# raznem/spp-rl

Measured on AMD Instinct MI355X. Metric: env-steps/sec (rollout+update) SPP-SAC Hopper-v2, higher is better.
Workload: dtype fp32

## Files before the change

include/spprl.h:

```cpp
#ifndef SPPRL_H
#define SPPRL_H
#include <stdint.h>

#ifdef __cplusplus
extern "C" {
#endif

typedef int sppStatus;
enum {
  SPP_OK = 0,
  SPP_E_INVALID_ARG = 1,
  SPP_E_SHAPE = 2,
  SPP_E_OOM = 3,
  SPP_E_HIP = 4,
  SPP_E_STATE = 5,
  SPP_E_RCCL = 6
};

const char* sppGetLastError(void);
int sppGetVersion(void);

typedef struct sppMT19937* sppMTHandle;
sppStatus sppMTCreate(sppMTHandle* out, uint32_t seed);
sppStatus sppMTRandint(sppMTHandle h, int64_t high, int64_t n, int64_t* out_host);
// ... 122 lines not shown
enum { SPP_BUCKET_CRITIC = 0, SPP_BUCKET_ACTOR = 1, SPP_BUCKET_ACM = 2, SPP_BUCKET_ALL = 3 };
sppStatus sppAllReduceGrads(sppAgentHandle h, int bucket, int world, void* rccl_comm, void* stream);
sppStatus sppCommAllReduceSum(void* rccl_comm, void* buf_dev, int64_t count, int dtype, void* stream);
sppStatus sppCommAllGather(void* rccl_comm, const void* send_dev, void* recv_dev, int64_t bytes, void* stream);

sppStatus sppAcmRegressStep(sppAgentHandle h, const float* x, const float* y, int B, float* loss_dev,
                            void* stream);
sppStatus sppAcmRegressGrads(sppAgentHandle h, const float* x, const float* y, int B, float* loss_dev,
                             void* stream);
sppStatus sppAcmRegressApply(sppAgentHandle h, void* stream);
sppStatus sppAcmSgd(sppAgentHandle h, const float* x_dev, const float* y_dev, int nsteps, int bs, float* loss_sum,
                    void* stream);
sppStatus sppAcmSgdEpoch(sppAgentHandle h, const float* x_dev, const float* y_dev, int nrows, int bs,
                         float* loss_sum, void* stream);
sppStatus sppAcmSgdStatus(sppAgentHandle h, int* timed_out_host);
sppStatus sppAcmSgdStatusAsync(sppAgentHandle h, int* timed_out_pinned, void* stream);
int sppAcmSgdMaxBatch(sppAgentHandle h);
int sppAcmSgdWorkgroups(sppAgentHandle h, int bs);
sppStatus sppReplayGatherAcm(sppReplayHandle h, const int64_t* idx_dev, int B, float* x, float* y, void* stream);
sppStatus sppReplaySetAcmColumns(sppReplayHandle h, const int* cols_host, int n);

sppStatus sppAgentSetTiming(sppAgentHandle h, int enable);
sppStatus sppAgentStageSplit(sppAgentHandle h, int* bits_out);
sppStatus sppAgentGetTiming(sppAgentHandle h, double* ms_out , int64_t* count_out );

sppStatus sppPolicyAct(sppAgentHandle h, const float* obs , int E, const float* eps ,
                       const float* noise , float act_noise, int mode, int denormalize_actor_out,
                       float* target_state_out , float* env_action_out , void* stream);

sppStatus sppSynthEnvStep(const float* A , const float* obs , const float* action ,
                          int E, int ob, int ac, float* next_obs, float* reward, void* stream);

sppStatus sppRandUniform(float* out_dev, int64_t n, const float* lo_dev, const float* hi_dev, int period,
                         uint64_t seed, uint64_t offset, void* stream);
sppStatus sppEpisodeAccum(const float* rew, const uint8_t* end, int E, float* ep_ret, double* sums, void* stream);
sppStatus sppSynthEnvReset(float* obs , const uint8_t* mask, int E, int ob, uint64_t seed,
                           uint64_t offset, void* stream);

sppStatus sppObsNormalize(const float* x, int64_t rows, int ob, const float* lo, const float* hi, const float* mean,
                          const float* std, int min_max, int inverse, float* out, void* stream);

sppStatus sppGaeScan(const float* rew, const float* v, const float* v_next, const uint8_t* done,
                     const uint8_t* end, int64_t T, int64_t E, double gamma, double lam, int mode, float* q_out,
                     float* adv, void* stream);
sppStatus sppPpoClipLoss(const float* lp_old, const float* lp_new, const float* adv, int B, float eps, float* grad,
                         float* out2, void* stream);
// ... 61 lines not shown
```

spp-rl_amd/csrc/api.hip:

```cpp
#include <dlfcn.h>
#include <stdarg.h>
#include <stdio.h>
#include <string.h>

#include <algorithm>
#include <memory>
#include <string>
#include <vector>

#include "../../include/spprl.h"
#include "internal.h"
#include "layout.h"
#include "replay.h"
#include "sac_kernels.h"
#include "host.h"

#include "optim.hip"
#include "replay.hip"
#include "stats.hip"
#include "sac.hip"
#include "ddpg.hip"
#include "kset.h"
#ifdef SPP_SINGLE_TU
#include "ks_dw.hip"
// ... 683 lines not shown
  DevArray<PackJob> d_pj;
  std::vector<TabSeg> tab;
  int tab_floats = 0;
  ActorDev actor{};
  CriticDev critic[2]{}, targ[2]{};
  AcmDev acm{};
  const float4* acm_W1n = nullptr;
  BAcmDev bacm{};
  ActorDev actor_targ{};
  const float4 *bacm_W1n = nullptr, *bacm_W21n = nullptr;
  BAcmScratch bz{};
  float *RBH = nullptr, *RBH1 = nullptr, *RS21 = nullptr, *RBP1 = nullptr, *RPZ = nullptr, *RPZ21 = nullptr;
  DevArray<float> scratch;
  float *S = nullptr, *S2 = nullptr, *ACT = nullptr, *AENV = nullptr, *R = nullptr, *DN = nullptr, *EPS1 = nullptr,
        *EPS2 = nullptr;
  float *H1[2] = {}, *H2[2] = {}, *D1[2] = {}, *D2[2] = {}, *DQ[2] = {};
  float *AH1 = nullptr, *AH2 = nullptr, *AD1 = nullptr, *AD2 = nullptr, *ADH = nullptr;
  float *Z1 = nullptr, *Z2 = nullptr, *T3 = nullptr, *part = nullptr;
  float *aux = nullptr;
  float* GAD = nullptr;
  uint64_t* MASK = nullptr;
  bool minq_split = false;
  int stage_split = 0;
  float *THD = nullptr, *SCA = nullptr, *SLP = nullptr;
  AcmScratch mq{};
  float *RX = nullptr, *RZ1 = nullptr, *RZ2 = nullptr, *RP1 = nullptr, *RP2 = nullptr, *RP3 = nullptr;
  DwSet dws[2];
  DevArray<AdamJob> d_adam;
  int cur_B = -1;
  float* w3p[2] = {};
  int64_t w3p_stride = 0;
  float* alpha_grad = nullptr;
  DevArray<float> sgd_slab;
  DevArray<int> sgd_sync;
  int sgd_max_wg = -1;
  bool timing = false;
  std::vector<hipEvent_t> tev[5];
  size_t tused[5] = {0, 0, 0, 0, 0};
};

static void tmark(sppAgent* a, int kind, hipStream_t st) {
  if (!a->timing) return;
  auto& v = a->tev[kind];
  if (a->tused[kind] == v.size()) {
    hipEvent_t e;
    hipEventCreate(&e);
// ... 360 lines not shown
  for (int i = 0; i < (a->ddpg ? 1 : 2); ++i) {
    NetBufs& n = a->net[SPP_NET_CRITIC1 + i];
    jobs[i] = AdamJob{n.p, n.g, n.m, n.v, a->net[SPP_NET_CRITIC1_TARG + i].p, n.n};
  }
  NetBufs& na = a->net[SPP_NET_ACTOR];
  jobs[2] = AdamJob{na.p, na.g, na.m, na.v, a->ddpg ? a->net[SPP_NET_ACTOR_TARG].p : nullptr, na.n};
  NetBufs& nm = a->net[SPP_NET_ACM];
  jobs[3] = AdamJob{nm.p, nm.g, nm.m, nm.v, nullptr, nm.n};
  if (!a->d_adam.ptr) SPP_CHECK_HIP(a->d_adam.alloc(4));
  SPP_CHECK_HIP(hipMemcpy(a->d_adam.ptr, jobs, sizeof(jobs), hipMemcpyHostToDevice));
  return SPP_OK;
}

static void launch_adam(sppAgent* a, int first, int count, int64_t n, int64_t step, float lr, float tau,
                        hipStream_t st) {
  const double bc1 = 1.0 - std::pow(0.9, (double)step), bc2s = std::sqrt(1.0 - std::pow(0.999, (double)step));
  hipLaunchKernelGGL(k_adam, dim3(std::max(1, std::min(cdiv(n, 256 * 4), 1024)), count), dim3(256), 0, st,
                     (const AdamJob*)(a->d_adam.ptr + first), (float)(-(lr / bc1)), (float)bc2s, tau);
}

constexpr int kStageWGPerCU = 3;
constexpr int kStageSplitAll = 7;
constexpr int kStageSplitDefault = kStageSplitAll;
static int stage_grid(sppAgent* a, int Bp) {
  return std::max(1, std::min(cdiv(Bp / 32, kWavesPerWG), kStageWGPerCU * a->num_cu));
}

static SacArgs make_args(sppAgent* a, int B) {
  SacArgs p{};
  p.B = B;
  p.Bp = (int)round_up(B, 32);
  p.inv_B = 1.f / (float)B;
  p.S = a->S; p.S2 = a->S2; p.ACT = a->ACT; p.AENV = a->AENV; p.R = a->R; p.DN = a->DN;
  p.EPS1 = a->EPS1; p.EPS2 = a->EPS2;
  p.min_max = a->cfg.min_max_denormalize;
  p.lo = a->lo; p.hi = a->hi; p.mean = a->mean; p.std = a->std;
  p.actor_lim = a->limits.ptr;
  p.acm_lim = a->limits.ptr + a->cfg.aout;
  p.gamma = a->cfg.gamma;
  p.custom_loss = a->cfg.custom_loss;
  p.norm_closs = a->cfg.norm_closs;
  p.alpha = a->alpha_f32;
  p.actor = a->actor;
  for (int i = 0; i < 2; ++i) {
    p.critic[i] = a->critic[i];
    p.targ[i] = a->targ[i];
// ... 75 lines not shown
  KernelSet ks;
  SPP_REQUIRE(find_kset(cfg->algo, cfg->ob, cfg->aout, cfg->ac, cfg->acm_critic != 0, cfg->mlp_bf16 != 0, &ks),
              SPP_E_SHAPE, "no kernel instantiation for algo %d (ob=%d, aout=%d, ac=%d, bf16=%d)", cfg->algo, cfg->ob,
              cfg->aout, cfg->ac, cfg->mlp_bf16);
  SPP_CHECK_HIP(hipSetDevice(device));
  auto a = std::make_unique<sppAgent>();
  a->cfg = *cfg;
  a->device = device;
  a->ks = ks;
  hipDeviceProp_t prop;
  SPP_CHECK_HIP(hipGetDeviceProperties(&prop, device));
  a->num_cu = prop.multiProcessorCount;
  {
    const char* t = getenv("SPP_SAC_TEAM");
    a->team_ok = !(t && t[0] == '0');
    const char* m = getenv("SPP_MINQ_SPLIT");
    a->minq_split = ks.actor_fwd && ks.actor_minq && ks.actor_bwd && !(m && m[0] == '0');
    const char* g = getenv("SPP_STAGE_SPLIT");
    const int want = g ? atoi(g) : kStageSplitDefault;
    const bool tab_fits = 128 + 3 * round_up(std::max(cfg->aout, 1), 32) + round_up(std::max(cfg->ac, 1), 32) <= kStageTab;
    const bool have = ks.heads_stage && ks.trunk_bwd && ks.trunk_fwd_a && ks.squash_a && ks.critics_a &&
                      ks.trunk_fwd_c && ks.squash_c && ks.critic_rest;
    if (a->minq_split && have && tab_fits) a->stage_split = want & kStageSplitAll;
  }
  const int ob = cfg->ob, aout = cfg->aout, ac = cfg->ac;
  a->cin = ob + (cfg->acm_critic ? ac : aout);
  a->ddpg = cfg->algo == SPP_ALGO_DDPG_ACM || cfg->algo == SPP_ALGO_DDPG;
  a->plain = cfg->algo == SPP_ALGO_SAC || cfg->algo == SPP_ALGO_DDPG;
  const bool dd = a->ddpg;
  a->lay[SPP_NET_ACTOR] = dd ? ddpg_actor_layout(ob, aout) : sac_actor_layout(ob, aout);
  if (dd) a->lay[SPP_NET_ACTOR_TARG] = a->lay[SPP_NET_ACTOR];
  a->lay[SPP_NET_CRITIC1] = a->lay[SPP_NET_CRITIC1_TARG] = critic_layout(a->cin);
  if (!dd) a->lay[SPP_NET_CRITIC2] = a->lay[SPP_NET_CRITIC2_TARG] = critic_layout(a->cin);
  if (!dd) a->lay[SPP_NET_ACM] = acm_layout(2 * ob, ac);
  else if (!a->plain) a->lay[SPP_NET_ACM] = bacm_layout(2 * ob, ac);
  a->Bmax = cfg->max_batch;
  const int64_t Bp = round_up(cfg->max_batch, 32);
  SPP_REQUIRE((int64_t)Bp * 256 * 4 < ((int64_t)1 << 31), SPP_E_SHAPE, "max_batch %d too large (31-bit buffer offsets)",
              cfg->max_batch);
  a->Bpmax = (int)Bp;
  const int64_t ntiles = Bp / 32;
  const int64_t per = Bp;
  int64_t total = 0;
  auto take = [&](int64_t rows) { int64_t o = total; total += rows * per; return o; };
  const int64_t oS = take(ob), oS2 = take(ob), oACT = take(aout), oAENV = take(ac), oR = take(1), oDN = take(1),
                oE1 = take(aout), oE2 = take(aout);
// ... 150 lines not shown
  hipLaunchKernelGGL(k_stage_batch, dim3(cdiv(s.Bp, 256)), dim3(256), 0, st, s);
  a->cur_B = bt->B;
  return SPP_OK;
}

static sppStatus critic_grads_staged(sppAgentHandle a, float* losses, hipStream_t st) {
  SPP_REQUIRE(!a->ddpg, SPP_E_STATE, "not a SAC_AcM agent");
  const int B = a->cur_B;
  SPP_REQUIRE(B > 0, SPP_E_STATE, "no staged batch");
  sppStatus s = check_ready(a);
  if (s) return s;
  if (a->dws[0].B != B) {
    s = build_dw(a, 0, B);
    if (s) return s;
  }
  launch_pack(a, PJ_ACTOR, PJ_LISTS, st);
  SacArgs p = make_args(a, B);
  const int grid = sac_critic_grid(a, p.Bp);
  tmark(a, 0, st);
  const bool team = phase_team(a, p.Bp);
  if (!team && (a->stage_split & 4)) {
    hipLaunchKernelGGL(a->ks.trunk_fwd_c, dim3(tile_grid(a, p.Bp)), dim3(256), 0, st, p, a->mq);
    hipLaunchKernelGGL(a->ks.squash_c, dim3(stage_grid(a, p.Bp)), dim3(256), 0, st, stage_args(a, p), a->mq);
    hipLaunchKernelGGL(a->ks.critic_rest, dim3(grid), dim3(256), 0, st, p);
  } else {
    hipLaunchKernelGGL(team ? a->ks.critic_team : a->ks.critic, dim3(grid), dim3(team ? 64 * kTeamCritic : 256), 0, st, p);
  }
  tmark(a, 0, st);
  SPP_CHECK_HIP(hipGetLastError());
  tmark(a, 2, st);
  launch_dw(a, 0, 0, st);
  tmark(a, 2, st);
  hipLaunchKernelGGL(k_finalize_critic, dim3(1), dim3(kFinThreads), 0, st, (const float*)a->part, p.Bp / 32, B, losses);
  SPP_CHECK_HIP(hipGetLastError());
  return SPP_OK;
}

sppStatus sppSacAcmCriticGrads(sppAgentHandle a, const sppBatch* bt, const float* eps_next, float* losses,
                               void* stream) {
  SPP_REQUIRE(a, SPP_E_INVALID_ARG, "null");
  if (bt) {
    sppStatus s = stage(a, bt, eps_next, nullptr, S(stream));
    if (s) return s;
  } else if (eps_next) {
    const int Bp = (int)round_up(a->cur_B, 32);
    SPP_REQUIRE(a->cur_B > 0, SPP_E_STATE, "no staged batch");
    hipLaunchKernelGGL(k_eps_copy_fm, dim3(cdiv((int64_t)a->cfg.aout * Bp, 256)), dim3(256), 0, S(stream), eps_next,
// ... 7 lines not shown
  a->steps[1] += 1;
  tmark(a, 3, S(stream));
  launch_adam(a, 0, 2, a->net[SPP_NET_CRITIC1].n, a->steps[1], a->cfg.critic_lr, a->cfg.tau, S(stream));
  tmark(a, 3, S(stream));
  SPP_CHECK_HIP(hipGetLastError());
  return SPP_OK;
}

static sppStatus actor_grads(sppAgentHandle a, float* losses, hipStream_t st) {
  SPP_REQUIRE(!a->ddpg, SPP_E_STATE, "not a SAC_AcM agent");
  const int B = a->cur_B;
  SPP_REQUIRE(B > 0, SPP_E_STATE, "no staged batch");
  launch_pack(a, PJ_CRITIC, PJ_LISTS, st);
  SacArgs p = make_args(a, B);
  AcmScratch z{a->Z1, a->Z2, a->T3, a->GAD, a->MASK};
  const int grid = tile_grid(a, p.Bp);
  tmark(a, 1, st);
  const bool team = phase_team(a, p.Bp);
  if (!team && a->minq_split) {
    z = a->mq;
    if (a->stage_split & 2) {
      hipLaunchKernelGGL(a->ks.trunk_fwd_a, dim3(grid), dim3(256), 0, st, p, z);
      hipLaunchKernelGGL(a->ks.squash_a, dim3(stage_grid(a, p.Bp)), dim3(256), 0, st, stage_args(a, p), z);
      hipLaunchKernelGGL(a->ks.critics_a, dim3(grid), dim3(256), 0, st, p, z);
    } else {
      hipLaunchKernelGGL(a->ks.actor_fwd, dim3(grid), dim3(256), 0, st, p, z);
    }
    hipLaunchKernelGGL(k_minq_scan, dim3(1), dim3(kMinqScanThreads), 0, st, (const uint32_t*)z.CNT, z.OFF, z.NG, p.Bp / 32);
    hipLaunchKernelGGL(k_minq_scatter, dim3(cdiv(p.Bp, 256)), dim3(256), 0, st, (const uint8_t*)z.SEL,
                       (const uint32_t*)z.OFF, z.LIST[0], z.LIST[1], p.Bp);
    hipLaunchKernelGGL(a->ks.actor_minq, dim3(grid), dim3(256), 0, st, p, z);
    if (a->stage_split & 1) {
      hipLaunchKernelGGL(a->ks.heads_stage, dim3(stage_grid(a, p.Bp)), dim3(256), 0, st, stage_args(a, p), z);
      hipLaunchKernelGGL(a->ks.trunk_bwd, dim3(grid), dim3(256), 0, st, p, z);
    } else {
      hipLaunchKernelGGL(a->ks.actor_bwd, dim3(grid), dim3(256), 0, st, p, z);
    }
  } else {
    hipLaunchKernelGGL(team ? a->ks.actor_team : a->ks.actor, dim3(grid), dim3(team ? 64 * kTeamActor : 256), 0, st, p, z);
    if (a->ks.actor_heads) hipLaunchKernelGGL(a->ks.actor_heads, dim3(grid), dim3(256), 0, st, p, z);
  }
  tmark(a, 1, st);
  SPP_CHECK_HIP(hipGetLastError());
  tmark(a, 2, st);
  launch_dw(a, 0, 1, st);
  tmark(a, 2, st);
  hipLaunchKernelGGL(k_actor_partials, dim3(1), dim3(kFinThreads), 0, st, (const float*)a->part, p.Bp / 32, B, a->cfg.aout,
                     a->cfg.custom_loss, (double)a->cfg.target_entropy, a->alpha_grad ? a->alpha_grad : a->aux,
                     losses);
  SPP_CHECK_HIP(hipGetLastError());
  return SPP_OK;
}

sppStatus sppSacAcmActorGrads(sppAgentHandle a, const float* eps_cur, float* losses, void* stream) {
  SPP_REQUIRE(a, SPP_E_INVALID_ARG, "null");
  const int B = a->cur_B;
  SPP_REQUIRE(B > 0, SPP_E_STATE, "no staged batch");
  const int Bp = (int)round_up(B, 32);
  if (eps_cur)
    hipLaunchKernelGGL(k_eps_copy_fm, dim3(cdiv((int64_t)a->cfg.aout * Bp, 256)), dim3(256), 0, S(stream), eps_cur,
                       a->EPS2, a->cfg.aout, B, Bp);
  return actor_grads(a, losses, S(stream));
}

sppStatus sppAgentStageSplit(sppAgentHandle a, int* bits_out) {
  SPP_REQUIRE(a && bits_out, SPP_E_INVALID_ARG, "null");
  *bits_out = a->stage_split;
  return SPP_OK;
}

sppStatus sppAgentBindAlphaGrad(sppAgentHandle a, float* g) {
  SPP_REQUIRE(a, SPP_E_INVALID_ARG, "null");
  a->alpha_grad = g;
  return SPP_OK;
}

sppStatus sppSacAcmDrawEps(sppAgentHandle a, uint64_t seed, uint64_t counter, void* stream) {
  SPP_REQUIRE(a && a->cur_B > 0, SPP_E_STATE, "no staged batch");
  const int B = a->cur_B, Bp = (int)round_up(B, 32);
  SPP_REQUIRE((int64_t)a->cfg.aout * Bp < ((int64_t)1 << 31), SPP_E_SHAPE, "draw_eps: aout * Bp >= 2^31");
  const int64_t quads = (int64_t)a->cfg.aout * Bp / 4;
  hipLaunchKernelGGL(k_eps_fm, dim3(cdiv(quads, 256), 2), dim3(256), 0, S(stream), a->EPS1, a->cfg.aout, B, Bp, seed,
                     2 * counter, a->EPS2, 2 * counter + 1);
  SPP_CHECK_HIP(hipGetLastError());
  return SPP_OK;
}

sppStatus sppAgentReadEps(sppAgentHandle a, int which, float* out, void* stream) {
  SPP_REQUIRE(a && out && (which == 0 || which == 1), SPP_E_INVALID_ARG, "read_eps: bad args");
  SPP_REQUIRE(a->cur_B > 0, SPP_E_STATE, "no staged batch");
// ... 621 lines not shown
```

spp-rl_amd/csrc/kset.h:

```cpp
#pragma once
#include "sac.hip"
#include "sac_bf.h"
#include "ddpg.hip"
#include "sac_team.h"
#include "ddpg_team.h"

namespace spp {

struct KernelSet {
  void (*critic)(SacArgs);
  void (*actor)(SacArgs, AcmScratch);
  void (*actor_heads)(SacArgs, AcmScratch);
  void (*act)(SacArgs, ActArgs);
  void (*acmreg)(SacArgs, AcmRegArgs);
  void (*dcritic)(SacArgs, BAcmScratch);
  void (*dactor)(SacArgs, BAcmScratch);
  void (*dact)(SacArgs, ActArgs, BAcmScratch);
  void (*dreg)(SacArgs, BAcmRegArgs);
  void (*critic_team)(SacArgs);
  void (*actor_team)(SacArgs, AcmScratch);
  void (*act_team)(SacArgs, ActArgs);
  void (*dcritic_team)(SacArgs, BAcmScratch);
  void (*dactor_team)(SacArgs, BAcmScratch);
  void (*dact_team)(SacArgs, ActArgs, BAcmScratch);
  void (*actor_fwd)(SacArgs, AcmScratch);
  void (*actor_minq)(SacArgs, AcmScratch);
  void (*actor_bwd)(SacArgs, AcmScratch);
  void (*heads_stage)(SacArgs, AcmScratch);
  void (*trunk_bwd)(SacArgs, AcmScratch);
  void (*trunk_fwd_a)(SacArgs, AcmScratch);
  void (*squash_a)(SacArgs, AcmScratch);
  void (*critics_a)(SacArgs, AcmScratch);
  void (*trunk_fwd_c)(SacArgs, AcmScratch);
  void (*squash_c)(SacArgs, AcmScratch);
  void (*critic_rest)(SacArgs);
};

template <int OB, int AOUT, int AC, bool ACMC, bool BF = false>
KernelSet make_kset() {
  using C = Cfg<OB, AOUT, AC, ACMC, BF>;
  void (*heads)(SacArgs, AcmScratch) = nullptr;
  if constexpr (C::NB_PAIR > 2) heads = k_sac_actor_heads<C>;
  void (*critic)(SacArgs) = k_sac_critic_phase<C>;
#if SPP_BF16_TWO_TILES
  if constexpr (C::BF && C::ACMC && !C::F3) critic = k_sac_critic_phase2<C>;
#endif
  KernelSet ks{critic, k_sac_actor_phase<C>, heads, k_policy_act<C>, k_acm_regress<C>,
               nullptr, nullptr, nullptr, nullptr};
  if constexpr (!C::BF) {
    ks.actor_fwd = k_sac_actor_phase<C, true>;
    ks.actor_minq = k_sac_minq_backward<C>;
    ks.actor_bwd = k_sac_actor_heads<C, true>;
    if constexpr (C::NB_PAIR <= 2) {
      ks.heads_stage = k_sac_heads_stage<C>;
      ks.trunk_bwd = k_sac_actor_trunk_bwd<C>;
      ks.trunk_fwd_a = k_sac_trunk_fwd<C, true>;
      ks.squash_a = k_sac_squash_stage<C, true>;
      ks.critics_a = k_sac_actor_phase<C, true, true>;
      ks.trunk_fwd_c = k_sac_trunk_fwd<C, false>;
      ks.squash_c = k_sac_squash_stage<C, false>;
      ks.critic_rest = k_sac_critic_phase<C, true>;
    }
  }
  return ks;
}
template <int OB, int AOUT, int AC, bool ACMC>
KernelSet make_dkset() {
  using D = DCfg<OB, AOUT, AC, ACMC>;
  return {nullptr, nullptr, nullptr, nullptr, nullptr,
          k_ddpg_critic_phase<D>, k_ddpg_actor_phase<D>, k_ddpg_policy_act<D>, k_bacm_regress<D>};
}

#define SPP_KSET_CASE(mk, o, a, c)                                     \
  if (ob == o && aout == a && ac == c) {                               \
    *ks = acmc ? mk<o, a, c, true>() : mk<o, a, c, false>();           \
    return true;                                                       \
  }

bool kset_sac_hopper(int ob, int aout, int ac, bool acmc, KernelSet* ks);
bool kset_sac_hcheetah(int ob, int aout, int ac, bool acmc, KernelSet* ks);
bool kset_sac_ant(int ob, int aout, int ac, bool acmc, KernelSet* ks);
bool kset_sac_small(int ob, int aout, int ac, bool acmc, KernelSet* ks);
bool kset_ddpg(int ob, int aout, int ac, bool acmc, KernelSet* ks);
bool kset_ddpg_ant(int ob, int aout, int ac, bool acmc, KernelSet* ks);
// ... 6 lines not shown
```

spp-rl_amd/csrc/sac.hip:

```cpp
#pragma once
#include "sac_kernels.h"

namespace spp {

constexpr float kLog2 = 0.69314718055994530942f;
constexpr float kLogSqrt2Pi = 0.91893853320467274178f;

template <int OB_, int AOUT_, int AC_, bool ACMC_, bool BF_ = false>
struct Cfg {
  static constexpr int OB = OB_, AOUT = AOUT_, AC = AC_;
  static constexpr bool ACMC = ACMC_;
  static constexpr bool BF = BF_;
  static constexpr bool F3 = !BF_ || SPP_BF16_FUSE3;
  static constexpr int NB_OB = blocks_of(OB);
  static constexpr int NB_AOUT = blocks_of(AOUT);
  static constexpr int NB_H2 = blocks_of(2 * AOUT);
  static constexpr int NB_PAIR = (AOUT + 15) / 16;
  static constexpr int CA = ACMC ? AC : AOUT;
  static constexpr int NB_CA = blocks_of(CA);
  static constexpr int NB_CIN = NB_OB + NB_CA;
  static constexpr int NB_ACMIN = NB_OB + NB_AOUT;
  static constexpr uint64_t RV_X = rv_nat(OB, NB_OB);
  static constexpr uint64_t RV_H = rv_nat(256, 8);
  static constexpr uint64_t RV_CIN = rv_cat(OB, NB_OB, CA, NB_CA);
// ... 457 lines not shown
        const float u = fadd_rn(mu, fmul_rn(e, sc));
        float lpj;
        if constexpr (F) {
          lpj = -0.5f * e * e - ls - kLogSqrt2Pi;
        } else {
          const float d = fsub_rn(u, mu);
          const float var = fmul_rn(sc, sc);
          lpj = fsub_rn(fsub_rn(fdiv_rn(-fmul_rn(d, d), 2.f * var), logf(sc)), kLogSqrt2Pi);
        }
        const float cj = 2.f * fsub_rn(fsub_rn(kLog2, u), t_softplus<F>(-2.f * u));
        lp += ok ? lpj : 0.f;
        corr += ok ? cj : 0.f;
        const float a = fmul_rn(t_tanh<F>(u), actor_lim<true>(p, L.tbl, jj));
        const float ad = denorm<true>(p, L.tbl, jj, a);
        if (ok) L.pl[j0 * 32] = ad;
      }
    }
  SPP_XLANE_SYNC();
  const float tot = lp + __shfl_xor(lp, 32, 64);
  const float tc = corr + __shfl_xor(corr, 32, 64);
  return fsub_rn(tot, tc);
}

template <class C, bool STAGED = false>
__global__ __launch_bounds__(256, 1) void k_sac_critic_phase(SacArgs p) {
  __shared__ __attribute__((aligned(16))) float smem[kWavesPerWG * kLdsPerWave];
  __shared__ __attribute__((aligned(16))) float tbl[kTabMax];
  __shared__ __attribute__((aligned(16))) float s_dq[kWavesPerWG][32];
  SPP_TP_INIT();
  load_table(p, tbl);
  const int w = threadIdx.x >> 6, lane = threadIdx.x & 63;
  float* big = smem + w * kLdsPerWave;
  float* small = big + kSmallRow * 32;
  const int ntiles = p.Bp / 32;
  const int ld = p.Bp;
  const float alpha = *p.alpha;
  float w3a[4] = {0.f, 0.f, 0.f, 0.f}, w3b[4] = {0.f, 0.f, 0.f, 0.f}, b3a = 0.f, b3b = 0.f;
  for (int tile = blockIdx.x * kWavesPerWG + w; tile < ntiles; tile += gridDim.x * kWavesPerWG) {
    const Lane L = make_lane(big, small, tbl, ld, tile * 32 + (lane & 31));
    const int b = L.b;
    const bool valid = b < p.B;
    uint64_t d0 = 0, d1 = 0, d2 = 0, d3 = 0;
    float lp2;
    f32x16 tin[C::NB_CIN];
    if constexpr (STAGED) {
      SPP_TP(0);
      load_cat_gg<C::NB_OB, C::NB_CA>(tin, p.S2, C::OB, p.SCA, C::CA, L.ld4, L.vo);
      lp2 = p.SLP[b];
    } else {
      SPP_TP(0);
      actor_trunk<C, false>(p.actor, p.S2, C::OB * L.ld4, L, nullptr, nullptr, d0, d1, d2, d3);
      {
        f32x16 hd[C::NB_PAIR];
        load_pair<C>(hd, big);
        lp2 = squash_write<C, true>(p, hd, p.EPS1, L);
      }
      SPP_TP(4);
      if constexpr (C::ACMC) {
        f32x16 xin[C::NB_ACMIN];
        load_cat_gl<C::NB_OB, C::NB_AOUT>(xin, p.S2, C::OB * L.ld4, C::OB, L.ld4, L.vo, big, C::AOUT);
        acm_forward<C, false>(p, xin, L, nullptr, nullptr, nullptr);
        load_cat_gl<C::NB_OB, C::NB_CA>(tin, p.S2, C::OB * L.ld4, C::OB, L.ld4, L.vo, small, C::AC);
      } else {
        load_cat_gl<C::NB_OB, C::NB_CA>(tin, p.S2, C::OB * L.ld4, C::OB, L.ld4, L.vo, big, C::AOUT);
      }
    }
    SPP_TP(5);
    const float q1t = critic_forward<C, false, 6>(p.targ[0], tin, L, nullptr, nullptr, d0, d1, d2, d3);
    const float q2t = critic_forward<C, false, 8>(p.targ[1], tin, L, nullptr, nullptr, d0, d1, d2, d3);
    const float notdone = 1.f - p.DN[b];
    const float y = fadd_rn(p.R[b], fmul_rn(p.gamma * notdone, fsub_rn(fminf(q1t, q2t), alpha * lp2)));
    float lq0 = 0.f, lq1 = 0.f;
#pragma unroll 1
    for (int i = 0; i < 2; ++i) {
      uint64_t m1lo = 0, m1hi = 0, m2lo = 0, m2hi = 0;
      f32x16 xin[C::NB_CIN];
      load_cat_gg<C::NB_OB, C::NB_CA>(xin, p.S, C::OB, C::ACMC ? p.AENV : p.ACT, C::CA, L.ld4, L.vo);
      const CriticDev& Q = p.critic[i];
      SPP_TP(10);
      const float q = critic_forward<C, true, 11, C::F3>(Q, xin, L, p.H1[i], C::F3 ? nullptr : p.H2[i], m1lo, m1hi,
                                                        m2lo, m2hi);
      const float diff = fsub_rn(q, y);
      const float dq = valid ? fmul_rn(2.f * diff, p.inv_B) : 0.f;
      const float lqi = (valid && L.h == 0) ? diff * diff : 0.f;
      if (i == 0) lq0 = lqi; else lq1 = lqi;
      if constexpr (!C::F3) {
        if (L.h == 0) p.DQ[i][b] = dq;
      } else {
      if (L.h == 0) s_dq[w][L.s] = dq;
      SPP_XLANE_SYNC();
#pragma unroll
      for (int k = 0; k < 4; ++k) {
        const int u = lane + 64 * k;
        const float* row = big + u * 32;
        float acc = 0.f;
#pragma unroll 8
        for (int j = 0; j < 32; ++j) {
          const int s2 = (j + u) & 31;
          acc = fmaf(row[s2], s_dq[w][s2], acc);
        }
        if (i == 0) w3a[k] += acc;
        else w3b[k] += acc;
      }
      const float dsum = wave_sum(L.h == 0 ? dq : 0.f);
      if (i == 0) b3a += dsum;
      else b3b += dsum;
      SPP_XLANE_SYNC();
      }
      const rsrc_t d2r = rsrc(p.D2[i]);
      const float* w3 = tbl + Q.tw3;
      const rsrc_t d1r = rsrc(p.D1[i]);
      auto epi1 = [&](int ob, const f32x16& acc) {
#pragma unroll
        for (int q2 = 0; q2 < 16; ++q2)
          op_st<C::BF>(d1r, 32 * ob + ru(q2), L.ld4, L.vo, getbit(m1lo, m1hi, ob, q2) ? acc[q2] : 0.f);
      };
      if constexpr (C::GEN_CD2) {
        const int ld4 = L.ld4;
        const uint32_t vo = L.vo;
        auto st2 = [=](int ur, float v) { op_st<C::BF>(d2r, ur, ld4, vo, v); };
        Delta2Gen<8, decltype(st2)> g{w3, L.h4, m2lo, m2hi, dq, st2, {}};
        SPP_TP(13);
        dense_gen<8>(Q.W2T, nullptr, g, epi1);
      } else {
#pragma unroll 1
        for (int ob = 0; ob < 8; ++ob) {
          float tv[16];
          tvals(w3, ob, L.h4, tv);
#pragma unroll
          for (int q2 = 0; q2 < 16; ++q2) {
            const int ur = 32 * ob + ru(q2);
            const float v = getbit(m2lo, m2hi, ob, q2) ? dq * tv[q2] : 0.f;
            L.bl[ur * 32] = v;
            op_st<C::BF>(d2r, ur, L.ld4, L.vo, v);
          }
        }
        SPP_TP(13);
        dense_lds<8, C::BF>(Q.W2T, big, nullptr, epi1);
      }
    }
    SPP_TP(14);
    const float s0 = wave_sum(lq0), s1 = wave_sum(lq1);
    if (lane == 0) {
      p.part[tile * kParts + 0] = s0;
      p.part[tile * kParts + 1] = s1;
    }
    SPP_TP(15);
  }
  if constexpr (C::F3) {
    const int64_t wg = (int64_t)blockIdx.x * kWavesPerWG + w;
    float* o0 = p.W3P[0] + wg * p.w3p_stride;
    float* o1 = p.W3P[1] + wg * p.w3p_stride;
#pragma unroll
    for (int k = 0; k < 4; ++k) {
      o0[lane + 64 * k] = w3a[k];
      o1[lane + 64 * k] = w3b[k];
    }
    if (lane == 0) {
      o0[256] = b3a;
      o1[256] = b3b;
    }
  }
  SPP_TP_FLUSH();
}

struct AcmScratch {
  float *Z1, *Z2, *T3;
  float* GAD;
  uint64_t* MASK;
  uint8_t* SEL;
  uint64_t* CM;
  uint32_t *CNT, *OFF;
  int* NG;
  int* LIST[2];
  float* DCA[2];
// ... 167 lines not shown
      dca[ib][q] = fadd_rn(fadd_rn(0.f, v1), v2);
    }
}

template <class C>
__device__ __forceinline__ void actor_trunk_backward(const SacArgs& p, const Lane& L, const f32x16 (&hd)[C::NB_PAIR],
                                                     uint64_t a1lo, uint64_t a1hi, uint64_t a2lo, uint64_t a2hi) {
  dense<C::NB_PAIR, C::RV_PAIR, C::BF>(p.actor.WhT, 8, hd, nullptr, [&](int ob, const f32x16& acc) {
#pragma unroll
    for (int q = 0; q < 16; ++q) {
      const int ur = 32 * ob + ru(q);
      const float v = getbit(a2lo, a2hi, ob, q) ? acc[q] : 0.f;
      L.bl[ur * 32] = v;
      op_st<C::BF>(rsrc(p.AD2), ur, L.ld4, L.vo, v);
    }
  });
  dense_lds<8, C::BF>(p.actor.W2T, L.img, nullptr, [&](int ob, const f32x16& acc) {
#pragma unroll
    for (int q = 0; q < 16; ++q)
      op_st<C::BF>(rsrc(p.AD1), 32 * ob + ru(q), L.ld4, L.vo, getbit(a1lo, a1hi, ob, q) ? acc[q] : 0.f);
  });
}

template <class C, bool SPLIT = false, bool STAGED = false>
__global__ __launch_bounds__(256, 1) void k_sac_actor_phase(SacArgs p, AcmScratch z) {
  static_assert(SPLIT || !STAGED, "the stage split cuts the split phase");
  __shared__ float smem[kWavesPerWG * kLdsPerWave];
  __shared__ __attribute__((aligned(16))) float tbl[kTabMax];
  SPP_TP_INIT();
  load_table(p, tbl);
  const int w = threadIdx.x >> 6, lane = threadIdx.x & 63;
  float* big = smem + w * kLdsPerWave;
  float* small = big + kSmallRow * 32;
  const int ntiles = p.Bp / 32;
  const int ld = p.Bp;
  const float alpha = *p.alpha;
  for (int tile = blockIdx.x * kWavesPerWG + w; tile < ntiles; tile += gridDim.x * kWavesPerWG) {
    const Lane L = make_lane(big, small, tbl, ld, tile * 32 + (lane & 31));
    const int b = L.b;
    const bool valid = b < p.B;
    const float g_lp = valid ? alpha * p.inv_B : 0.f;
    uint64_t a1lo = 0, a1hi = 0, a2lo = 0, a2hi = 0;
    f32x16 hd[C::NB_PAIR];
    float lp;
    f32x16 cin[C::NB_CIN];
    constexpr bool kWide = C::NB_PAIR > 2;
    if constexpr (STAGED) {
      SPP_TP(26);
      load_cat_gg<C::NB_OB, C::NB_CA>(cin, p.S, C::OB, p.SCA, C::CA, L.ld4, L.vo);
      lp = p.SLP[b];
    } else {
      SPP_TP(26);
      actor_trunk<C, true>(p.actor, p.S, C::OB * L.ld4, L, p.AH1, p.AH2, a1lo, a1hi, a2lo, a2hi);
      SPP_TP(27);
      load_pair<C>(hd, big);
      lp = squash_write<C>(p, hd, p.EPS2, L);
      SPP_TP(28);
      constexpr bool kParkHeads = kWide || SPLIT;
      if constexpr (kParkHeads) {
#pragma unroll
        for (int ib = 0; ib < C::NB_PAIR; ++ib)
#pragma unroll
          for (int r = 0; r < 8; ++r) {
            const int j0 = 16 * ib + r;
            if (j0 + 8 * L.h < C::AOUT) {
              fm_st(rsrc(p.ADH), j0, L.ld4, L.vp, hd[ib][r]);
              fm_st(rsrc(p.ADH), C::AOUT + j0, L.ld4, L.vp, hd[ib][r + 8]);
            }
          }
      }
      if constexpr (C::ACMC) {
        f32x16 xin[C::NB_ACMIN];
        load_cat_gl<C::NB_OB, C::NB_AOUT>(xin, p.S, C::OB * L.ld4, C::OB, L.ld4, L.vo, big, C::AOUT);
        acm_forward<C, true>(p, xin, L, z.Z1, z.Z2, z.T3);
        load_cat_gl<C::NB_OB, C::NB_CA>(cin, p.S, C::OB * L.ld4, C::OB, L.ld4, L.vo, small, C::AC);
      } else {
        load_cat_gl<C::NB_OB, C::NB_CA>(cin, p.S, C::OB * L.ld4, C::OB, L.ld4, L.vo, big, C::AOUT);
      }
    }
    SPP_TP(29);
    uint64_t ma0 = 0, ma1 = 0, ma2 = 0, ma3 = 0, mb0 = 0, mb1 = 0, mb2 = 0, mb3 = 0;
    const float q1 = critic_forward<C, false>(p.critic[0], cin, L, nullptr, nullptr, ma0, ma1, ma2, ma3);
    const float q2 = critic_forward<C, false>(p.critic[1], cin, L, nullptr, nullptr, mb0, mb1, mb2, mb3);
    const float qmin = fminf(q1, q2);
    const float gq = valid ? -p.inv_B : 0.f;
    const float dqa = q1 < q2 ? gq : (q1 == q2 ? 0.5f * gq : 0.f);
    const float dqb = q2 < q1 ? gq : (q1 == q2 ? 0.5f * gq : 0.f);
    SPP_TP(19);
    if constexpr (SPLIT) {
      const int sel = valid ? (int)(q1 <= q2) | ((int)(q2 <= q1) << 1) : 0;
      if (L.h == 0) z.SEL[b] = (uint8_t)sel;
      uint4* cm0 = reinterpret_cast<uint4*>(z.CM + ((int64_t)b * 2 + L.h) * 4);
      uint4* cm1 = reinterpret_cast<uint4*>(z.CM + (((int64_t)ld + b) * 2 + L.h) * 4);
      cm0[0] = make_uint4((uint32_t)ma0, (uint32_t)(ma0 >> 32), (uint32_t)ma1, (uint32_t)(ma1 >> 32));
      cm0[1] = make_uint4((uint32_t)ma2, (uint32_t)(ma2 >> 32), (uint32_t)ma3, (uint32_t)(ma3 >> 32));
      cm1[0] = make_uint4((uint32_t)mb0, (uint32_t)(mb0 >> 32), (uint32_t)mb1, (uint32_t)(mb1 >> 32));
      cm1[1] = make_uint4((uint32_t)mb2, (uint32_t)(mb2 >> 32), (uint32_t)mb3, (uint32_t)(mb3 >> 32));
      const int n1 = __popcll(__ballot(L.h == 0 && (sel & 1))), n2 = __popcll(__ballot(L.h == 0 && (sel & 2)));
      if constexpr (!STAGED) {
        uint64_t* mk = z.MASK + (int64_t)tile * 4 * 64 + lane;
        mk[0] = a1lo;
        mk[64] = a1hi;
        mk[128] = a2lo;
        mk[192] = a2hi;
      }
      const float ps = wave_sum((valid && L.h == 0) ? fsub_rn(alpha * lp, qmin) : 0.f);
      const float pl = wave_sum((valid && L.h == 0) ? lp : 0.f);
      if (lane == 0) {
        z.CNT[tile] = (uint32_t)n1 | ((uint32_t)n2 << 16);
        p.part[tile * kParts + 2] = ps;
        p.part[tile * kParts + 4] = pl;
      }
      continue;
    }
    f32x16 dca[C::NB_CA];
#pragma unroll
    for (int ib = 0; ib < C::NB_CA; ++ib) dca[ib] = zero16();
#pragma unroll 1
    for (int i = 0; i < 2; ++i) {
      const CriticDev& Q = p.critic[i];
// ... 742 lines not shown
```

spp-rl_amd/spprl/_lib.py:

```python
import ctypes
import os

import torch

HERE = os.path.dirname(os.path.abspath(__file__))
LIB_PATH = os.environ.get("SPPRL_LIB") or os.path.join(HERE, "libspprl.so")

(SPP_NET_ACTOR, SPP_NET_CRITIC1, SPP_NET_CRITIC2, SPP_NET_CRITIC1_TARG, SPP_NET_CRITIC2_TARG, SPP_NET_ACM,
 SPP_NET_ACTOR_TARG) = range(7)
SPP_ALGO_SAC_ACM, SPP_ALGO_DDPG_ACM, SPP_ALGO_SAC, SPP_ALGO_DDPG = 1, 2, 3, 4
SPP_BUCKET_CRITIC, SPP_BUCKET_ACTOR, SPP_BUCKET_ACM, SPP_BUCKET_ALL = range(4)
SPP_COMM_ID_BYTES = 128
SPP_DP1_REUSE_BRACKET = 0x100
NUM_LOSSES = 8

c_int, c_int64, c_uint32, c_uint64, c_float, c_void_p = (ctypes.c_int, ctypes.c_int64, ctypes.c_uint32,
                                                         ctypes.c_uint64, ctypes.c_float, ctypes.c_void_p)


class SppError(RuntimeError):
    pass


class AgentConfig(ctypes.Structure):
# ... 61 lines not shown
    "sppSacAcmUpdate": (c_int, [c_void_p, P(Batch), c_void_p, c_void_p, c_void_p, c_void_p]),
    "sppSacAcmCriticGrads": (c_int, [c_void_p, P(Batch), c_void_p, c_void_p, c_void_p]),
    "sppSacAcmCriticApply": (c_int, [c_void_p, c_void_p]),
    "sppSacAcmActorGrads": (c_int, [c_void_p, c_void_p, c_void_p, c_void_p]),
    "sppSacAcmActorApply": (c_int, [c_void_p, c_void_p, c_void_p]),
    "sppAgentStageFromReplay": (c_int, [c_void_p, c_void_p, c_void_p, c_int, c_void_p]),
    "sppAgentStagePost": (c_int, [c_void_p, c_int, c_int, c_void_p]),
    "sppSacAcmUpdateStaged": (c_int, [c_void_p, c_uint64, c_uint64, c_void_p, c_void_p]),
    "sppAcmRegressStep": (c_int, [c_void_p, c_void_p, c_void_p, c_int, c_void_p, c_void_p]),
    "sppPolicyAct": (c_int, [c_void_p, c_void_p, c_int, c_void_p, c_void_p, c_float, c_int, c_int, c_void_p,
                             c_void_p, c_void_p]),
    "sppAgentBindAlphaGrad": (c_int, [c_void_p, c_void_p]),
    "sppSacAcmDrawEps": (c_int, [c_void_p, c_uint64, c_uint64, c_void_p]),
    "sppAgentReadEps": (c_int, [c_void_p, c_int, c_void_p, c_void_p]),
    "sppAgentImageCount": (c_int, [c_void_p, c_int, c_void_p]),
    "sppAgentUnpackImage": (c_int, [c_void_p, c_int, c_int, c_void_p, c_void_p]),
    "sppAcmRegressGrads": (c_int, [c_void_p, c_void_p, c_void_p, c_int, c_void_p, c_void_p]),
    "sppAcmRegressApply": (c_int, [c_void_p, c_void_p]),
    "sppReplayGatherAcm": (c_int, [c_void_p, c_void_p, c_int, c_void_p, c_void_p, c_void_p]),
    "sppReplaySetAcmColumns": (c_int, [c_void_p, c_void_p, c_int]),
    "sppAgentSetTiming": (c_int, [c_void_p, c_int]),
    "sppAgentGetTiming": (c_int, [c_void_p, c_void_p, c_void_p]),
    "sppAgentStageSplit": (c_int, [c_void_p, P(c_int)]),
    "sppSynthEnvStep": (c_int, [c_void_p, c_void_p, c_void_p, c_int, c_int, c_int, c_void_p, c_void_p, c_void_p]),
    "sppDdpgAcmUpdate": (c_int, [c_void_p, P(Batch), c_void_p, c_void_p]),
    "sppDdpgAcmCriticGrads": (c_int, [c_void_p, P(Batch), c_void_p, c_void_p]),
    "sppDdpgAcmCriticApply": (c_int, [c_void_p, c_void_p]),
    "sppDdpgAcmActorGrads": (c_int, [c_void_p, c_void_p, c_void_p]),
    "sppDdpgAcmActorApply": (c_int, [c_void_p, c_void_p]),
    "sppOnpCreate": (c_int, [P(c_void_p), P(OnPolicyConfig), c_int]),
    "sppOnpDestroy": (c_int, [c_void_p]),
    "sppOnpNetSize": (c_int, [c_void_p, c_int, P(c_int64)]),
    "sppOnpBindNet": (c_int, [c_void_p, c_int, c_void_p, c_void_p, c_void_p, c_void_p]),
    "sppOnpSetLimits": (c_int, [c_void_p, c_void_p]),
    "sppOnpValue": (c_int, [c_void_p, c_void_p, c_int, c_void_p, c_void_p]),
    "sppOnpCriticGrads": (c_int, [c_void_p, c_void_p, c_void_p, c_int, c_void_p, c_void_p]),
    "sppOnpCriticApply": (c_int, [c_void_p, c_void_p]),
    "sppOnpActorGrads": (c_int, [c_void_p, c_void_p, c_void_p, c_void_p, c_void_p, c_void_p, c_int, c_void_p,
                                 c_void_p]),
    "sppOnpActorApply": (c_int, [c_void_p, c_void_p]),
    "sppOnpTdAdvantage": (c_int, [c_void_p, c_void_p, c_void_p, c_void_p, c_void_p, c_int, c_float, c_void_p,
                                  c_void_p, c_void_p, c_void_p]),
    "sppOnpPgActorGrads": (c_int, [c_void_p] * 7 + [c_int, c_void_p, c_void_p]),
    "sppOnpAct": (c_int, [c_void_p, c_void_p, c_int, c_void_p, c_void_p, c_void_p, c_void_p]),
    "sppOnpRolloutAct": (c_int, [c_void_p, c_void_p, c_int, c_void_p, c_void_p, c_uint64, c_uint64, c_int, c_void_p,
                                 c_void_p, c_void_p, c_void_p, c_void_p]),
# ... 83 lines not shown
```

Before: 458,000.

## Split twin critics across paired waves in staged critic and actor phases

Adds a pair form of the staged critic and actor-phase kernels. In it, neighbouring waves each evaluate one of the two critics for the same tile and swap their Q values through LDS after a block barrier. Per-critic fc3 partial slabs are remapped so each critic's slabs stay contiguous. The aim is to halve the serial per-wave critic work and double wave-level parallelism when the batch has few tiles. The cost is extra barriers, LDS traffic and duplicated input loads. By default only the critic-rest pair path is enabled; the actor-phase pair needs an environment bit.

```diff
diff --git a/include/spprl.h b/include/spprl.h
--- a/include/spprl.h
+++ b/include/spprl.h
@@ -168,6 +168,7 @@
 
 sppStatus sppAgentSetTiming(sppAgentHandle h, int enable);
 sppStatus sppAgentStageSplit(sppAgentHandle h, int* bits_out);
+sppStatus sppAgentCriticPairs(sppAgentHandle h, int* bits_out);
 sppStatus sppAgentGetTiming(sppAgentHandle h, double* ms_out , int64_t* count_out );
 
 sppStatus sppPolicyAct(sppAgentHandle h, const float* obs , int E, const float* eps ,
diff --git a/spp-rl_amd/csrc/api.hip b/spp-rl_amd/csrc/api.hip
--- a/spp-rl_amd/csrc/api.hip
+++ b/spp-rl_amd/csrc/api.hip
@@ -729,6 +729,7 @@
   uint64_t* MASK = nullptr;
   bool minq_split = false;
   int stage_split = 0;
+  int critic_pairs = 0;
   float *THD = nullptr, *SCA = nullptr, *SLP = nullptr;
   AcmScratch mq{};
   float *RX = nullptr, *RZ1 = nullptr, *RZ2 = nullptr, *RP1 = nullptr, *RP2 = nullptr, *RP3 = nullptr;
@@ -1135,6 +1136,7 @@
 constexpr int kStageWGPerCU = 3;
 constexpr int kStageSplitAll = 7;
 constexpr int kStageSplitDefault = kStageSplitAll;
+constexpr int kCriticPairsDefault = 1;
 static int stage_grid(sppAgent* a, int Bp) {
   return std::max(1, std::min(cdiv(Bp / 32, kWavesPerWG), kStageWGPerCU * a->num_cu));
 }
@@ -1256,6 +1258,10 @@
     const bool have = ks.heads_stage && ks.trunk_bwd && ks.trunk_fwd_a && ks.squash_a && ks.critics_a &&
                       ks.trunk_fwd_c && ks.squash_c && ks.critic_rest;
     if (a->minq_split && have && tab_fits) a->stage_split = want & kStageSplitAll;
+    const char* cp = getenv("SPP_CRITIC_PAIRS");
+    const int wantp = cp ? atoi(cp) : kCriticPairsDefault;
+    if ((a->stage_split & 4) && ks.critic_rest_pair) a->critic_pairs |= wantp & 1;
+    if ((a->stage_split & 2) && ks.critics_a_pair) a->critic_pairs |= wantp & 2;
   }
   const int ob = cfg->ob, aout = cfg->aout, ac = cfg->ac;
   a->cin = ob + (cfg->acm_critic ? ac : aout);
@@ -1452,7 +1458,7 @@
   if (!team && (a->stage_split & 4)) {
     hipLaunchKernelGGL(a->ks.trunk_fwd_c, dim3(tile_grid(a, p.Bp)), dim3(256), 0, st, p, a->mq);
     hipLaunchKernelGGL(a->ks.squash_c, dim3(stage_grid(a, p.Bp)), dim3(256), 0, st, stage_args(a, p), a->mq);
-    hipLaunchKernelGGL(a->ks.critic_rest, dim3(grid), dim3(256), 0, st, p);
+    hipLaunchKernelGGL((a->critic_pairs & 1) ? a->ks.critic_rest_pair : a->ks.critic_rest, dim3(grid), dim3(256), 0, st, p);
   } else {
     hipLaunchKernelGGL(team ? a->ks.critic_team : a->ks.critic, dim3(grid), dim3(team ? 64 * kTeamCritic : 256), 0, st, p);
   }
@@ -1506,7 +1512,7 @@
     if (a->stage_split & 2) {
       hipLaunchKernelGGL(a->ks.trunk_fwd_a, dim3(grid), dim3(256), 0, st, p, z);
       hipLaunchKernelGGL(a->ks.squash_a, dim3(stage_grid(a, p.Bp)), dim3(256), 0, st, stage_args(a, p), z);
-      hipLaunchKernelGGL(a->ks.critics_a, dim3(grid), dim3(256), 0, st, p, z);
+      hipLaunchKernelGGL((a->critic_pairs & 2) ? a->ks.critics_a_pair : a->ks.critics_a, dim3(grid), dim3(256), 0, st, p, z);
     } else {
       hipLaunchKernelGGL(a->ks.actor_fwd, dim3(grid), dim3(256), 0, st, p, z);
     }
@@ -1550,6 +1556,12 @@
 sppStatus sppAgentStageSplit(sppAgentHandle a, int* bits_out) {
   SPP_REQUIRE(a && bits_out, SPP_E_INVALID_ARG, "null");
   *bits_out = a->stage_split;
+  return SPP_OK;
+}
+
+sppStatus sppAgentCriticPairs(sppAgentHandle a, int* bits_out) {
+  SPP_REQUIRE(a && bits_out, SPP_E_INVALID_ARG, "null");
+  *bits_out = a->critic_pairs;
   return SPP_OK;
 }
 
diff --git a/spp-rl_amd/csrc/kset.h b/spp-rl_amd/csrc/kset.h
--- a/spp-rl_amd/csrc/kset.h
+++ b/spp-rl_amd/csrc/kset.h
@@ -34,6 +34,8 @@
   void (*trunk_fwd_c)(SacArgs, AcmScratch);
   void (*squash_c)(SacArgs, AcmScratch);
   void (*critic_rest)(SacArgs);
+  void (*critics_a_pair)(SacArgs, AcmScratch);
+  void (*critic_rest_pair)(SacArgs);
 };
 
 template <int OB, int AOUT, int AC, bool ACMC, bool BF = false>
@@ -60,6 +62,8 @@
       ks.trunk_fwd_c = k_sac_trunk_fwd<C, false>;
       ks.squash_c = k_sac_squash_stage<C, false>;
       ks.critic_rest = k_sac_critic_phase<C, true>;
+      ks.critics_a_pair = k_sac_actor_phase<C, true, true, true>;
+      ks.critic_rest_pair = k_sac_critic_phase<C, true, true>;
     }
   }
   return ks;
diff --git a/spp-rl_amd/csrc/sac.hip b/spp-rl_amd/csrc/sac.hip
--- a/spp-rl_amd/csrc/sac.hip
+++ b/spp-rl_amd/csrc/sac.hip
@@ -503,8 +503,25 @@
   return fsub_rn(tot, tc);
 }
 
-template <class C, bool STAGED = false>
+struct PairMap {
+  int c, j, P, K;
+};
+__device__ __forceinline__ PairMap pair_map(int ntiles) {
+  const int gw = __builtin_amdgcn_readfirstlane((int)(blockIdx.x * kWavesPerWG + (threadIdx.x >> 6)));
+  const int P = 2 * (int)gridDim.x;
+  return {gw & 1, gw >> 1, P, (ntiles + P - 1) / P};
+}
+using PairSlot = float[kWavesPerWG / 2][2][2][32];
+
+__device__ __forceinline__ float sac_target_y(const SacArgs& p, int b, float q1t, float q2t, float alpha, float lp2) {
+  const float notdone = 1.f - p.DN[b];
+  return fadd_rn(p.R[b], fmul_rn(p.gamma * notdone, fsub_rn(fminf(q1t, q2t), alpha * lp2)));
+}
+
+template <class C, bool STAGED = false, bool PAIR = false>
 __global__ __launch_bounds__(256, 1) void k_sac_critic_phase(SacArgs p) {
+  static_assert(STAGED || !PAIR, "the pair form starts at the target critics");
+  static_assert(C::F3 || !PAIR, "the pair form keeps the fused fc3 slabs");
   __shared__ __attribute__((aligned(16))) float smem[kWavesPerWG * kLdsPerWave];
   __shared__ __attribute__((aligned(16))) float tbl[kTabMax];
   __shared__ __attribute__((aligned(16))) float s_dq[kWavesPerWG][32];
@@ -517,14 +534,35 @@
   const int ld = p.Bp;
   const float alpha = *p.alpha;
   float w3a[4] = {0.f, 0.f, 0.f, 0.f}, w3b[4] = {0.f, 0.f, 0.f, 0.f}, b3a = 0.f, b3b = 0.f;
-  for (int tile = blockIdx.x * kWavesPerWG + w; tile < ntiles; tile += gridDim.x * kWavesPerWG) {
+  const PairMap pm = PAIR ? pair_map(ntiles) : PairMap{};
+  int tile = PAIR ? pm.j : blockIdx.x * kWavesPerWG + w;
+  for (int k = 0; PAIR ? k < pm.K : tile < ntiles; ++k, tile += PAIR ? pm.P : gridDim.x * kWavesPerWG) {
     const Lane L = make_lane(big, small, tbl, ld, tile * 32 + (lane & 31));
     const int b = L.b;
     const bool valid = b < p.B;
     uint64_t d0 = 0, d1 = 0, d2 = 0, d3 = 0;
     float lp2;
     f32x16 tin[C::NB_CIN];
-    if constexpr (STAGED) {
+    float q1t, q2t;
+    if constexpr (PAIR) {
+      const bool active = tile < ntiles;
+      __shared__ PairSlot s_q;
+      float* slot = &s_q[w >> 1][k & 1][0][0];
+      float qt = 0.f;
+      if (active) {
+        SPP_TP(0);
+        load_cat_gg<C::NB_OB, C::NB_CA>(tin, p.S2, C::OB, p.SCA, C::CA, L.ld4, L.vo);
+        lp2 = p.SLP[b];
+        SPP_TP(5);
+        qt = critic_forward<C, false, 6>(p.targ[pm.c], tin, L, nullptr, nullptr, d0, d1, d2, d3);
+        if (L.h == 0) slot[32 * pm.c + L.s] = qt;
+      }
+      __syncthreads();
+      if (!active) continue;
+      const float qo = slot[32 * (pm.c ^ 1) + L.s];
+      q1t = pm.c ? qo : qt;
+      q2t = pm.c ? qt : qo;
+    } else if constexpr (STAGED) {
       SPP_TP(0);
       load_cat_gg<C::NB_OB, C::NB_CA>(tin, p.S2, C::OB, p.SCA, C::CA, L.ld4, L.vo);
       lp2 = p.SLP[b];
@@ -546,14 +584,17 @@
         load_cat_gl<C::NB_OB, C::NB_CA>(tin, p.S2, C::OB * L.ld4, C::OB, L.ld4, L.vo, big, C::AOUT);
       }
     }
-    SPP_TP(5);
-    const float q1t = critic_forward<C, false, 6>(p.targ[0], tin, L, nullptr, nullptr, d0, d1, d2, d3);
-    const float q2t = critic_forward<C, false, 8>(p.targ[1], tin, L, nullptr, nullptr, d0, d1, d2, d3);
-    const float notdone = 1.f - p.DN[b];
-    const float y = fadd_rn(p.R[b], fmul_rn(p.gamma * notdone, fsub_rn(fminf(q1t, q2t), alpha * lp2)));
+    if constexpr (!PAIR) {
+      SPP_TP(5);
+      q1t = critic_forward<C, false, 6>(p.targ[0], tin, L, nullptr, nullptr, d0, d1, d2, d3);
+      q2t = critic_forward<C, false, 8>(p.targ[1], tin, L, nullptr, nullptr, d0, d1, d2, d3);
+    }
+    const float y = sac_target_y(p, b, q1t, q2t, alpha, lp2);
     float lq0 = 0.f, lq1 = 0.f;
+    const int i0 = PAIR ? pm.c : 0, i1 = PAIR ? pm.c + 1 : 2;
 #pragma unroll 1
-    for (int i = 0; i < 2; ++i) {
+    for (int i = i0; i < i1; ++i) {
+      const bool seta = PAIR ? (k & 1) == 0 : i == 0;
       uint64_t m1lo = 0, m1hi = 0, m2lo = 0, m2hi = 0;
       f32x16 xin[C::NB_CIN];
       load_cat_gg<C::NB_OB, C::NB_CA>(xin, p.S, C::OB, C::ACMC ? p.AENV : p.ACT, C::CA, L.ld4, L.vo);
@@ -580,11 +621,11 @@
           const int s2 = (j + u) & 31;
           acc = fmaf(row[s2], s_dq[w][s2], acc);
         }
-        if (i == 0) w3a[k] += acc;
+        if (seta) w3a[k] += acc;
         else w3b[k] += acc;
       }
       const float dsum = wave_sum(L.h == 0 ? dq : 0.f);
-      if (i == 0) b3a += dsum;
+      if (seta) b3a += dsum;
       else b3b += dsum;
       SPP_XLANE_SYNC();
       }
@@ -623,15 +664,15 @@
     SPP_TP(14);
     const float s0 = wave_sum(lq0), s1 = wave_sum(lq1);
     if (lane == 0) {
-      p.part[tile * kParts + 0] = s0;
-      p.part[tile * kParts + 1] = s1;
+      if (!PAIR || pm.c == 0) p.part[tile * kParts + 0] = s0;
+      if (!PAIR || pm.c == 1) p.part[tile * kParts + 1] = s1;
     }
     SPP_TP(15);
   }
   if constexpr (C::F3) {
     const int64_t wg = (int64_t)blockIdx.x * kWavesPerWG + w;
-    float* o0 = p.W3P[0] + wg * p.w3p_stride;
-    float* o1 = p.W3P[1] + wg * p.w3p_stride;
+    float* o0 = PAIR ? p.W3P[pm.c] + (int64_t)pm.j * p.w3p_stride : p.W3P[0] + wg * p.w3p_stride;
+    float* o1 = PAIR ? p.W3P[pm.c] + (int64_t)(pm.j + pm.P) * p.w3p_stride : p.W3P[1] + wg * p.w3p_stride;
 #pragma unroll
     for (int k = 0; k < 4; ++k) {
       o0[lane + 64 * k] = w3a[k];
@@ -845,9 +886,10 @@
   });
 }
 
-template <class C, bool SPLIT = false, bool STAGED = false>
+template <class C, bool SPLIT = false, bool STAGED = false, bool PAIR = false>
 __global__ __launch_bounds__(256, 1) void k_sac_actor_phase(SacArgs p, AcmScratch z) {
   static_assert(SPLIT || !STAGED, "the stage split cuts the split phase");
+  static_assert(STAGED || !PAIR, "the pair form is the staged kernel's");
   __shared__ float smem[kWavesPerWG * kLdsPerWave];
   __shared__ __attribute__((aligned(16))) float tbl[kTabMax];
   SPP_TP_INIT();
@@ -858,7 +900,9 @@
   const int ntiles = p.Bp / 32;
   const int ld = p.Bp;
   const float alpha = *p.alpha;
-  for (int tile = blockIdx.x * kWavesPerWG + w; tile < ntiles; tile += gridDim.x * kWavesPerWG) {
+  const PairMap pm = PAIR ? pair_map(ntiles) : PairMap{};
+  int tile = PAIR ? pm.j : blockIdx.x * kWavesPerWG + w;
+  for (int k = 0; PAIR ? k < pm.K : tile < ntiles; ++k, tile += PAIR ? pm.P : gridDim.x * kWavesPerWG) {
     const Lane L = make_lane(big, small, tbl, ld, tile * 32 + (lane & 31));
     const int b = L.b;
     const bool valid = b < p.B;
@@ -868,7 +912,26 @@
     float lp;
     f32x16 cin[C::NB_CIN];
     constexpr bool kWide = C::NB_PAIR > 2;
-    if constexpr (STAGED) {
+    uint64_t ma0 = 0, ma1 = 0, ma2 = 0, ma3 = 0, mb0 = 0, mb1 = 0, mb2 = 0, mb3 = 0;
+    float q1, q2;
+    if constexpr (PAIR) {
+      const bool active = tile < ntiles;
+      __shared__ PairSlot s_q;
+      float* slot = &s_q[w >> 1][k & 1][0][0];
+      if (active) {
+        SPP_TP(26);
+        load_cat_gg<C::NB_OB, C::NB_CA>(cin, p.S, C::OB, p.SCA, C::CA, L.ld4, L.vo);
+        q1 = critic_forward<C, false>(p.critic[pm.c], cin, L, nullptr, nullptr, ma0, ma1, ma2, ma3);
+        if (L.h == 0) slot[32 * pm.c + L.s] = q1;
+        uint4* cm = reinterpret_cast<uint4*>(z.CM + (((int64_t)pm.c * ld + b) * 2 + L.h) * 4);
+        cm[0] = make_uint4((uint32_t)ma0, (uint32_t)(ma0 >> 32), (uint32_t)ma1, (uint32_t)(ma1 >> 32));
+        cm[1] = make_uint4((uint32_t)ma2, (uint32_t)(ma2 >> 32), (uint32_t)ma3, (uint32_t)(ma3 >> 32));
+      }
+      __syncthreads();
+      if (!active || pm.c != 0) continue;
+      q2 = slot[32 + L.s];
+      lp = p.SLP[b];
+    } else if constexpr (STAGED) {
       SPP_TP(26);
       load_cat_gg<C::NB_OB, C::NB_CA>(cin, p.S, C::OB, p.SCA, C::CA, L.ld4, L.vo);
       lp = p.SLP[b];
@@ -902,9 +965,10 @@
       }
     }
     SPP_TP(29);
-    uint64_t ma0 = 0, ma1 = 0, ma2 = 0, ma3 = 0, mb0 = 0, mb1 = 0, mb2 = 0, mb3 = 0;
-    const float q1 = critic_forward<C, false>(p.critic[0], cin, L, nullptr, nullptr, ma0, ma1, ma2, ma3);
-    const float q2 = critic_forward<C, false>(p.critic[1], cin, L, nullptr, nullptr, mb0, mb1, mb2, mb3);
+    if constexpr (!PAIR) {
+      q1 = critic_forward<C, false>(p.critic[0], cin, L, nullptr, nullptr, ma0, ma1, ma2, ma3);
+      q2 = critic_forward<C, false>(p.critic[1], cin, L, nullptr, nullptr, mb0, mb1, mb2, mb3);
+    }
     const float qmin = fminf(q1, q2);
     const float gq = valid ? -p.inv_B : 0.f;
     const float dqa = q1 < q2 ? gq : (q1 == q2 ? 0.5f * gq : 0.f);
@@ -913,12 +977,14 @@
     if constexpr (SPLIT) {
       const int sel = valid ? (int)(q1 <= q2) | ((int)(q2 <= q1) << 1) : 0;
       if (L.h == 0) z.SEL[b] = (uint8_t)sel;
-      uint4* cm0 = reinterpret_cast<uint4*>(z.CM + ((int64_t)b * 2 + L.h) * 4);
-      uint4* cm1 = reinterpret_cast<uint4*>(z.CM + (((int64_t)ld + b) * 2 + L.h) * 4);
-      cm0[0] = make_uint4((uint32_t)ma0, (uint32_t)(ma0 >> 32), (uint32_t)ma1, (uint32_t)(ma1 >> 32));
-      cm0[1] = make_uint4((uint32_t)ma2, (uint32_t)(ma2 >> 32), (uint32_t)ma3, (uint32_t)(ma3 >> 32));
-      cm1[0] = make_uint4((uint32_t)mb0, (uint32_t)(mb0 >> 32), (uint32_t)mb1, (uint32_t)(mb1 >> 32));
-      cm1[1] = make_uint4((uint32_t)mb2, (uint32_t)(mb2 >> 32), (uint32_t)mb3, (uint32_t)(mb3 >> 32));
+      if constexpr (!PAIR) {
+        uint4* cm0 = reinterpret_cast<uint4*>(z.CM + ((int64_t)b * 2 + L.h) * 4);
+        uint4* cm1 = reinterpret_cast<uint4*>(z.CM + (((int64_t)ld + b) * 2 + L.h) * 4);
+        cm0[0] = make_uint4((uint32_t)ma0, (uint32_t)(ma0 >> 32), (uint32_t)ma1, (uint32_t)(ma1 >> 32));
+        cm0[1] = make_uint4((uint32_t)ma2, (uint32_t)(ma2 >> 32), (uint32_t)ma3, (uint32_t)(ma3 >> 32));
+        cm1[0] = make_uint4((uint32_t)mb0, (uint32_t)(mb0 >> 32), (uint32_t)mb1, (uint32_t)(mb1 >> 32));
+        cm1[1] = make_uint4((uint32_t)mb2, (uint32_t)(mb2 >> 32), (uint32_t)mb3, (uint32_t)(mb3 >> 32));
+      }
       const int n1 = __popcll(__ballot(L.h == 0 && (sel & 1))), n2 = __popcll(__ballot(L.h == 0 && (sel & 2)));
       if constexpr (!STAGED) {
         uint64_t* mk = z.MASK + (int64_t)tile * 4 * 64 + lane;
diff --git a/spp-rl_amd/spprl/_lib.py b/spp-rl_amd/spprl/_lib.py
--- a/spp-rl_amd/spprl/_lib.py
+++ b/spp-rl_amd/spprl/_lib.py
@@ -107,6 +107,7 @@
     "sppAgentSetTiming": (c_int, [c_void_p, c_int]),
     "sppAgentGetTiming": (c_int, [c_void_p, c_void_p, c_void_p]),
     "sppAgentStageSplit": (c_int, [c_void_p, P(c_int)]),
+    "sppAgentCriticPairs": (c_int, [c_void_p, P(c_int)]),
     "sppSynthEnvStep": (c_int, [c_void_p, c_void_p, c_void_p, c_int, c_int, c_int, c_void_p, c_void_p, c_void_p]),
     "sppDdpgAcmUpdate": (c_int, [c_void_p, P(Batch), c_void_p, c_void_p]),
     "sppDdpgAcmCriticGrads": (c_int, [c_void_p, P(Batch), c_void_p, c_void_p]),
```

Measured after the change: 467,100, median of 6. +2.0%, better.
